# MGI-tech-bioinformatics/SuperPlus

Hardware: AMD Instinct MI355X
Metric: k-mers/s (DF createDict stage: trim + canonical k-mer count + solid filter + spectrum + adjacency) (higher is better)
Workload: dtype u64

## Files before the change

superplus_amd/csrc/dfk.hip:

```cpp
#include "../../include/dfk.h"
#include "dfk_kernels.h"
#include "dfk_arena.h"

#include <algorithm>
#include <chrono>
#include <cstdarg>
#include <cstdio>
#include <cstdlib>
#include <cstring>
#include <atomic>
#include <fcntl.h>
#include <functional>
#include <new>
#include <string>
#include <sys/mman.h>
#include <sys/stat.h>
#include <unistd.h>
#include <condition_variable>
#include <memory>
#include <mutex>
#include <numeric>
#include <thread>
#include <vector>

// ... 201 lines not shown
    }
    DevBuf sums; int rc = c->alloc(sums, nblk * 8, "scan block sums"); if (rc) return rc;
    hipLaunchKernelGGL(k_scan_blocks, dim3((unsigned)nblk), dim3(SCAN_THREADS), 0, c->stream, in, out, n, (uint64_t*)sums.p);
    HIP_TRY(hipGetLastError());
    rc = device_scan(c, (const uint64_t*)sums.p, (uint64_t*)sums.p, nblk); if (rc) return rc;
    hipLaunchKernelGGL(k_scan_add, dim3((unsigned)nblk), dim3(SCAN_THREADS), 0, c->stream, out, n, (const uint64_t*)sums.p);
    HIP_TRY(hipGetLastError());
    HIP_TRY(hipStreamSynchronize(c->stream));
    c->release(sums);
    return 0;
}

struct BucketTable {
    uint32_t log2_nb = 0;
    DevBuf acc;
    DevBuf summ;
    DevBuf classes;
    DevBuf ovf_list; uint64_t n_ovf = 0;
    DevBuf class_hist;
    std::vector<uint64_t> h_class;
    uint64_t n_records = 0, n_inst = 0;
};
struct Partition {
    DevBuf records, base, ipre, items;
    uint64_t n_records = 0, n_inst = 0, n_items = 0;
    uint64_t nb = 0;
};

template <int K>
PartParams part_params(const dfk_ctx* c, uint32_t log2_nb, uint32_t log2_world, int64_t read_id0, uint32_t sub_lo, uint32_t sub_n)
{
    const uint32_t M = c->cfg.minimizer_len;
    return PartParams{M, (uint32_t)K - M + 1, log2_nb, log2_world, read_id0, sub_lo, sub_n,
                      sweep_class_mask(sub_lo, sub_n, log2_nb - log2_world)};
}

int table_totals(dfk_ctx* c, const DevBuf& acc, uint64_t nb, uint64_t* n_records, uint64_t* n_inst)
{
    DevBuf tot; int rc = c->alloc(tot, 16, "bucket totals"); if (rc) return rc;
    HIP_TRY(hipMemsetAsync(tot.p, 0, 16, c->stream));
    hipLaunchKernelGGL(k_sum_acc, dim3(1024), dim3(256), 0, c->stream, (const unsigned long long*)acc.p, nb, (unsigned long long*)tot.p);
    HIP_TRY(hipGetLastError());
    uint64_t h[2];
    HIP_TRY(hipMemcpyAsync(h, tot.p, 16, hipMemcpyDeviceToHost, c->stream));
    HIP_TRY(hipStreamSynchronize(c->stream));
    c->release(tot);
    *n_records = h[0]; *n_inst = h[1];
    return 0;
}

struct ScanJob {
    PartParams pp; ScanPlan plan;
    DevBuf ovf_tmp, d_n;
    DevBuf keys, keys2, fill, sub;
    uint64_t n_pieces = 0; bool count_due = false;
    hipEvent_t ev_scan = nullptr, ev_count = nullptr, ev_part[2] = {nullptr, nullptr};
    std::vector<std::pair<hipEvent_t, hipEvent_t>> ev;
    ~ScanJob()
    {
        for (auto& e : ev) { (void)hipEventDestroy(e.first); (void)hipEventDestroy(e.second); }
        for (hipEvent_t e : {ev_scan, ev_count, ev_part[0], ev_part[1]}) if (e) (void)hipEventDestroy(e);
    }
};

template <int K> bool scan_takes_ranges(const dfk_ctx* c) { return c->cfg.minimizer_len == 16; }

ScanSwitches scan_switches()
// ... 209 lines not shown
    hipLaunchKernelGGL(k_item_flags, dim3(g1), dim3(256), 0, c->stream, (const uint64_t*)P->ipre.p, nb, budget, (uint64_t*)flags.p);
    HIP_TRY(hipGetLastError());
    rc = device_scan(c, (const uint64_t*)flags.p, (uint64_t*)idx.p, nb + 1); if (rc) return rc;
    uint64_t tot[3];
    HIP_TRY(hipMemcpyAsync(&tot[0], (const uint64_t*)P->base.p + nb, 8, hipMemcpyDeviceToHost, c->stream));
    HIP_TRY(hipMemcpyAsync(&tot[1], (const uint64_t*)P->ipre.p + nb, 8, hipMemcpyDeviceToHost, c->stream));
    HIP_TRY(hipMemcpyAsync(&tot[2], (const uint64_t*)idx.p + nb, 8, hipMemcpyDeviceToHost, c->stream));
    HIP_TRY(hipStreamSynchronize(c->stream));
    P->n_records = tot[0]; P->n_inst = tot[1]; P->n_items = tot[2];
    rc = c->alloc(P->items, std::max<uint64_t>(1, P->n_items) * sizeof(ItemRange), "work items"); if (rc) return rc;
    hipLaunchKernelGGL(k_item_pairs, dim3((unsigned)((nb + 255) / 256)), dim3(256), 0, c->stream, (const uint64_t*)flags.p,
                       (const uint64_t*)idx.p, nb, (ItemRange*)P->items.p);
    HIP_TRY(hipGetLastError());
    HIP_TRY(hipStreamSynchronize(c->stream));
    c->release(rec); c->release(inst); c->release(flags); c->release(idx);
    return 0;
}

void release_pass(dfk_ctx* c, Partition* P)
{ c->release(P->records); c->release(P->base); c->release(P->ipre); c->release(P->items); }

template <int K> uint64_t item_budget(const dfk_ctx* c)
{
    constexpr uint64_t S = 1ull << CountCfg<K>::LOG2S;
    if (c->cfg.inst_per_item) return c->cfg.inst_per_item;
    if (c->distinct_per_inst <= 0.0) return 3 * S / 2;
    const double b = 0.367 * (double)S / c->distinct_per_inst;
    return (uint64_t)std::min(std::max(b, 0.5 * (double)S), 3.0 * (double)S);
}

struct ScatterJob { Partition P; DevBuf cur, d_bad; hipStream_t st = nullptr; hipEvent_t e0 = nullptr, e1 = nullptr; uint32_t lo = 0, n = 0; };

template <int K>
int scatter_launch(dfk_ctx* c, const Inputs& in, const BucketTable& T, uint32_t log2_world, int64_t read_id0, ScatterJob* J)
{
    const PartParams pp = part_params<K>(c, T.log2_nb, log2_world, read_id0, J->lo, J->n);
    HIP_TRY(hipEventRecord(J->e0, J->st));
    if (in.n_reads)
        hipLaunchKernelGGL(HIP_KERNEL_NAME(k_scatter_runs<K>), dim3((unsigned)((in.n_reads + 256ull * sweep_reads<K>() - 1) / (256ull * sweep_reads<K>()))),
                           dim3(256), 0, J->st,
                           in.packed, in.packed_bytes, in.base_off, (const uint32_t*)c->good_len.p, in.bc,
                           (int64_t)c->cfg.ign_bc_below, in.n_reads, pp, (const uint4*)T.summ.p, (const uint32_t*)T.classes.p,
                           (unsigned long long*)J->cur.p, J->P.n_records, (uint4*)J->P.records.p);
    HIP_TRY(hipGetLastError());
    HIP_TRY(hipEventRecord(J->e1, J->st));
    return 0;
}

template <int K>
int scatter_begin(dfk_ctx* c, const Inputs& in, const BucketTable& T, uint32_t log2_world, int64_t read_id0,
                  uint32_t sub_lo, uint32_t sub_n, ScatterJob* J, bool launch_now = true)
{
    Partition* P = &J->P;
    J->st = c->stream; J->lo = sub_lo; J->n = sub_n;
    const PartParams pp = part_params<K>(c, T.log2_nb, log2_world, read_id0, sub_lo, sub_n);
    const uint64_t budget = item_budget<K>(c);
    int rc = pass_tables(c, T.acc, T.log2_nb - log2_world, 1u << log2_world, sub_lo, sub_n, budget, P); if (rc) return rc;
    const uint64_t nb = P->nb;
    rc = c->alloc(J->cur, nb * 8, "bucket cursors"); if (rc) return rc;
    rc = c->alloc(P->records, P->n_records * 32, "super-k-mer records"); if (rc) return rc;
    rc = c->alloc(J->d_bad, 16, "scatter check"); if (rc) return rc;
    HIP_TRY(hipMemcpyAsync(J->cur.p, P->base.p, nb * 8, hipMemcpyDeviceToDevice, c->stream));
    HIP_TRY(hipMemsetAsync(J->d_bad.p, 0, 16, c->stream));
    if (!J->e0) { HIP_TRY(hipEventCreate(&J->e0)); HIP_TRY(hipEventCreate(&J->e1)); }
    (void)pp;
    if (launch_now) return scatter_launch<K>(c, in, T, log2_world, read_id0, J);
    return 0;
}

template <int K>
int scatter_end(dfk_ctx* c, const Inputs& in, const BucketTable& T, uint32_t log2_world, int64_t read_id0, ScatterJob* J)
{
    HIP_TRY(hipEventSynchronize(J->e1));
// ... 567 lines not shown
        DevBuf d_n; rc = c->alloc(d_n, 16, "probe counter"); if (rc) return rc;
        HIP_TRY(hipMemsetAsync(d_n.p, 0, 16, c->stream));
        for (const dfk_ctx::Part& pt : c->parts) {
            if (!pt.n) continue;
            if (listed) {
                if (pt.n_blist)
                    hipLaunchKernelGGL(HIP_KERNEL_NAME(k_adjacency_list<K>), dim3((unsigned)std::min<uint64_t>((pt.n_blist + 255) / 256, 16384)), dim3(256), 0,
                                       c->stream, (uint4*)pt.buf.p, (const uint32_t*)((const char*)pt.buf.p + pt.blist + 16), pt.n_blist,
                                       (const SetSlot*)c->set.p, c->set_mask, (unsigned long long*)d_n.p);
            } else
                hipLaunchKernelGGL(HIP_KERNEL_NAME(k_adjacency<K>), dim3((unsigned)std::min<uint64_t>((pt.n + 255) / 256, 8192)), dim3(256), 0,
                                   c->stream, (uint4*)pt.buf.p, pt.n, (const SetSlot*)c->set.p, c->set_mask, (unsigned long long*)d_n.p);
        }
        HIP_TRY(hipGetLastError());
        uint64_t np = 0;
        HIP_TRY(hipMemcpyAsync(&np, d_n.p, 8, hipMemcpyDeviceToHost, c->stream));
        HIP_TRY(hipStreamSynchronize(c->stream));
        c->st.adj_probes = np;
        c->release(d_n); c->release(c->set);
    }
    c->st.ms_adjacency = t.stop();
    TRACE("adjacency done");
    return 0;
}

uint32_t pick_log2_nb(uint64_t n_inst, uint32_t log2_world)
{
    static const uint64_t per = getenv("DFK_INST_PER_BUCKET") ? (uint64_t)atoll(getenv("DFK_INST_PER_BUCKET")) : 850;
    return dfk::pick_log2_nb(n_inst, log2_world, per);
}

PlanInputs plan_inputs(const dfk_ctx* c, const BucketTable& T, const CountRun& R, uint32_t sub_nb, uint32_t lo, bool overlap)
{
    static const double first_div = getenv("DFK_PLAN_FIRST") ? atof(getenv("DFK_PLAN_FIRST")) : 10.0;
    static const double growth = getenv("DFK_PLAN_GROWTH") ? atof(getenv("DFK_PLAN_GROWTH")) : 1.1;
    return PlanInputs{c->budget > c->held ? (double)(c->budget - c->held) : 0.0, sub_nb, lo, T.n_inst, T.n_records, R.inst_seen, R.solid_seen,
                      c->cfg.min_freq, c->seg_attempt, c->plan_derate, overlap, first_div, growth, g_trace};
}

struct StreamSwap {
    dfk_ctx* c; hipStream_t keep;
    StreamSwap(dfk_ctx* ctx, hipStream_t s) : c(ctx), keep(ctx->stream) { c->stream = s; }
    ~StreamSwap() { c->stream = keep; }
};

struct Prescan { BucketTable T; uint64_t n_inst = 0; float ms_trim = 0; };

template <int K>
int run_typed(dfk_ctx* c, const Inputs& in, Prescan* pre = nullptr)
{
    Timer total(c->stream);
    total.start();
    Timer t(c->stream);
    uint64_t n_inst = 0;
    int rc = 0;
    BucketTable T;
    if (pre) { n_inst = pre->n_inst; c->st.ms_trim = pre->ms_trim; T = std::move(pre->T); }
    else {
        t.start();
        TRACE("trim: %llu reads", (unsigned long long)in.n_reads);
        rc = stage_trim<K>(c, in, &n_inst); if (rc) return rc;
        c->st.ms_trim = t.stop();
        TRACE("trim done: %llu instances", (unsigned long long)n_inst);
    }
    c->st.n_reads = in.n_reads; c->st.n_inst = n_inst; c->n_reads = in.n_reads;
    if (!pre) {
        T.log2_nb = pick_log2_nb(n_inst, 0);
        rc = partition_count<K>(c, in, n_inst, 0, 0, &T); if (rc) return rc;
    }
    CountRun R;
    rc = count_run_begin(c, &R); if (rc) return rc;
    c->want_blist = true; c->pending_blist = -1;
    const uint32_t sub_nb = 1u << T.log2_nb;
    const uint32_t forced = (uint32_t)c->cfg.reserved[0];
    const uint32_t per_forced = forced ? std::max<uint32_t>(1, (sub_nb + forced - 1) / forced) : 0;
    const bool overlap = getenv("DFK_NO_OVERLAP") == nullptr;
    uint32_t n_passes = 0, retries = 0;
    c->seg_attempt = 0; c->distinct_per_inst = 0.0;
    struct Job { ScatterJob sj; Arena::PassBlock blk; uint64_t mark = 0; bool valid = false; };
    Job cur, nxt;
    auto drop_events = [&](Job& j) { if (j.sj.e0) { (void)hipEventDestroy(j.sj.e0); (void)hipEventDestroy(j.sj.e1); j.sj.e0 = j.sj.e1 = nullptr; } };
    static const double defer_below = getenv("DFK_DEFER_SWEEP_BELOW") ? atof(getenv("DFK_DEFER_SWEEP_BELOW")) : 1.0;
    auto start = [&](Job& j, uint32_t lo, uint32_t n, bool may_defer = false) -> int {
        j.sj = ScatterJob{}; j.mark = c->alloc_seq; j.valid = false;
        const bool defer = may_defer && (double)n < defer_below * (double)sub_nb;
        TRACE("pass range [%u, %u) of %u (%.1f %%), %.2f GB held of %.2f", lo, lo + n, sub_nb, 100.0 * n / sub_nb, c->held / 1e9, c->budget / 1e9);
        j.blk = Arena::PassBlock{};
        int r = c->alloc(j.blk.block, pass_block_bytes(n, sub_nb, T.n_records), "pass block");
        if (!r) { Arena::Current in_blk(c->arena, j.blk); StreamSwap sw(c, c->stream2); r = scatter_begin<K>(c, in, T, 0, 0, lo, n, &j.sj, !defer); }
        if (r) { (void)hipStreamSynchronize(c->stream2); c->release_since(j.mark); drop_events(j); return r; }
        if (defer) { ScatterJob* sj = &j.sj; c->after_count_launch = [c, &in, &T, sj]() { return scatter_launch<K>(c, in, T, 0, 0, sj); }; TRACE("  (its sweep starts behind k_count)"); }
        j.valid = true;
        return 0;
    };
    auto start_alone = [&](Job& j, uint32_t lo) -> int {
        for (;;) {
            const uint32_t n = forced ? std::min(per_forced, sub_nb - lo) : plan_range(plan_inputs(c, T, R, sub_nb, lo, overlap), c->arena.free_blocks(), nullptr);
            if (!forced && n < sub_nb - lo && (uint64_t)n * 1024 < sub_nb)
                return fail(DFK_E_NOMEM, "HBM budget too small: %.2f GB free of %.2f GB allows passes of %u of %u buckets",
                            (c->budget - c->held) / 1e9, c->budget / 1e9, n, sub_nb);
            const int r = start(j, lo, n);
            if (r != DFK_E_NOMEM || forced || n <= 16 || ++retries > 12) return r;
            c->plan_derate *= 0.7;
            TRACE("out of HBM (%s): planning smaller passes", g_err.c_str());
        }
    };
    rc = start_alone(cur, 0); if (rc) return rc;
    while (cur.valid) {
        const uint32_t lo = cur.sj.lo, n = cur.sj.n, nlo = lo + n;
        rc = scatter_end<K>(c, in, T, 0, 0, &cur.sj); if (rc) return rc;
        const dfk_stats st0 = c->st;
        rc = count_snapshot(c, &R, false); if (rc) return rc;
        { Arena::Current in_blk(c->arena, cur.blk); rc = count_prepare<K>(c, cur.sj.P, R, barcode_words(c, in.bc != nullptr)); }
        nxt.valid = false;
        if (!rc && overlap && nlo < sub_nb) {
            const Partition& P = cur.sj.P;
            (void)P;
            const RunningPass rp{cur.blk.block.bytes, cur.sj.P.n_inst, n, c->arena.offset_of(cur.blk.block)};
            const uint32_t n2 = forced ? std::min(per_forced, sub_nb - nlo) : plan_range(plan_inputs(c, T, R, sub_nb, nlo, overlap), c->arena.free_blocks(), &rp);
            if (n2) {
                const int r2 = start(nxt, nlo, n2, true);
                if (r2 && r2 != DFK_E_NOMEM) return r2;
            }
        }
// ... 698 lines not shown
```

superplus_amd/csrc/dfk_kernels.h:

```cpp
#pragma once
#include <type_traits>
#include "dfk_device.h"
#include "dfk_fallback.h"
#include "dfk_scan_plan.h"

namespace dfk {

template <int K>
__global__ void __launch_bounds__(256)
k_trim(const uint8_t* __restrict__ pq, const uint64_t* __restrict__ pq_off, uint64_t pq_nbytes,
       const uint64_t* __restrict__ base_off, uint64_t packed_bytes, const uint32_t* __restrict__ read_len,
       uint64_t n_reads, uint32_t min_qual, uint32_t* __restrict__ good_len,
       unsigned long long* __restrict__ n_inst, unsigned int* __restrict__ bad,
       unsigned long long* __restrict__ sum_good)
{
    unsigned long long mine = 0, good = 0;
    bool any_bad = false;
    for (uint64_t r = (uint64_t)blockIdx.x * blockDim.x + threadIdx.x; r < n_reads; r += (uint64_t)gridDim.x * blockDim.x) {
        uint32_t gl = 0;
        uint64_t p = pq_off[r], end = pq_off[r + 1];
        uint32_t idx = 0, run = 0;
        const uint64_t b0 = base_off[r], b1 = base_off[r + 1];
        bool ok = p <= end && end <= pq_nbytes && b0 <= b1 && b1 <= packed_bytes && b1 - b0 >= ((uint64_t)read_len[r] + 3) / 4;
        if (!ok) end = p;
// ... 36 lines not shown
        if (gl > rl) gl = rl;
        good_len[r] = gl;
        good += gl;
        if (gl >= (uint32_t)K + 1) mine += gl - K + 1;
    }
    __shared__ unsigned long long sh[2][4];
    __shared__ unsigned int sh_bad;
    if (threadIdx.x == 0) sh_bad = 0;
    __syncthreads();
#pragma unroll
    for (int d = 32; d > 0; d >>= 1) { mine += __shfl_down(mine, d, 64); good += __shfl_down(good, d, 64); }
    if ((threadIdx.x & 63) == 0) { sh[0][threadIdx.x >> 6] = mine; sh[1][threadIdx.x >> 6] = good; }
    if (any_bad) atomicOr(&sh_bad, 1u);
    __syncthreads();
    if (threadIdx.x == 0) {
        unsigned long long a0 = sh[0][0] + sh[0][1] + sh[0][2] + sh[0][3], a1 = sh[1][0] + sh[1][1] + sh[1][2] + sh[1][3];
        if (a0) atomicAdd(n_inst, a0);
        if (a1) atomicAdd(sum_good, a1);
        if (sh_bad) atomicOr(bad, 1u);
    }
}

struct PartParams {
    uint32_t M;
    uint32_t W;
    uint32_t log2_nb;
    uint32_t log2_world;
    int64_t  read_id0;
    uint32_t sub_lo;
    uint32_t sub_n;
    uint32_t class_mask;
};

constexpr uint32_t SWEEP_CLASSES = 32;
__host__ __device__ inline uint32_t sweep_class_of(uint32_t local_bucket, uint32_t log2_local)
{ return log2_local > 5 ? local_bucket >> (log2_local - 5) : local_bucket; }
__host__ __device__ inline uint32_t sweep_class_mask(uint32_t sub_lo, uint32_t sub_n, uint32_t log2_local)
{
    if (sub_n == 0) return 0u;
    const uint32_t a = sweep_class_of(sub_lo, log2_local), b = sweep_class_of(sub_lo + sub_n - 1, log2_local);
    const uint32_t upto_b = b >= 31 ? 0xFFFFFFFFu : ((1u << (b + 1)) - 1u);
    return upto_b & ~((1u << a) - 1u);
}

constexpr uint32_t SUMMARY_OVERFLOW = 15;

__device__ __forceinline__ uint32_t pass_local(uint32_t bucket, const PartParams& pp)
{
    const uint32_t ls = pp.log2_nb - pp.log2_world;
    const uint32_t d = (bucket & ((1u << ls) - 1u)) - pp.sub_lo;
    return d < pp.sub_n ? (bucket >> ls) * pp.sub_n + d : 0xFFFFFFFFu;
}

__device__ __forceinline__ uint32_t bucket_of(uint32_t minhash, const PartParams& pp)
{
    const uint32_t b = (minhash * 0x9E3779B1u) >> (32 - pp.log2_nb);
    return ((b & ((1u << pp.log2_world) - 1u)) << (pp.log2_nb - pp.log2_world)) | (b >> pp.log2_world);
}
constexpr int PART_QCAP = 8;

template <int K>
__device__ __forceinline__ void emit_record(const uint32_t* __restrict__ words, uint64_t n_words, uint64_t bit0,
                                            uint32_t s0, uint32_t nk, uint32_t bucket, uint32_t gl, int32_t tag,
                                            uint64_t dst_index, uint4* __restrict__ records)
{
    const bool hp = s0 > 0;
    const bool hs = s0 + nk + (uint32_t)K <= gl;
    uint64_t bo = bit0 + 2ull * (hp ? s0 - 1 : 0);
    uint64_t wi = bo >> 5; uint32_t sh = (uint32_t)bo & 31u;
    uint32_t w[7];
#pragma unroll
    for (int i = 0; i < 7; ++i) w[i] = (wi + i < n_words) ? words[wi + i] : 0u;
    uint32_t o[6];
#pragma unroll
    for (int i = 0; i < 6; ++i) o[i] = alignbit(w[i + 1], w[i], sh);
    if (!hp) {
#pragma unroll
        for (int i = 5; i > 0; --i) o[i] = (o[i] << 2) | (o[i - 1] >> 30);
// ... 58 lines not shown
    const uint64_t bit0 = byte0 * 8;
    int32_t tag = -1;
    if (bc && (int64_t)r + pp.read_id0 >= ign_bc_below) tag = bc[r];

    const uint32_t mmask = M == 16 ? 0xFFFFFFFFu : ((1u << (2 * M)) - 1u);
    const uint32_t rsh = 2 * (M - 1);
    uint32_t f = 0, rc = 0;
    uint32_t P = 0;
    uint32_t bi = 0;
    uint32_t cur_b = 0, cur_s0 = 0, cur_nk = 0;
    uint32_t qn = 0;

    uint64_t wi = bit0 >> 5;
    uint64_t filled_to = wi;
    auto fill = [&]() {
        uint32_t w[PART_RING];
#pragma unroll
        for (int k = 0; k < PART_RING; ++k) w[k] = filled_to + k < n_words ? words[filled_to + k] : 0u;
#pragma unroll
        for (int k = 0; k < PART_RING; ++k) ring[((filled_to + k) & (PART_RING - 1)) * PART_THREADS + tid] = w[k];
        filled_to += PART_RING;
    };
    uint32_t wbits, wnext = 0;
    if (!WRITE) { fill(); wbits = ring[(wi & (PART_RING - 1)) * PART_THREADS + tid]; }
    else { wbits = wi < n_words ? words[wi] : 0u; wnext = wi + 1 < n_words ? words[wi + 1] : 0u; }
    uint32_t wpos = (uint32_t)bit0 & 31u;
    uint32_t sfx_next = 0xFFFFFFFFu;

    auto close_run = [&]() {
        if (WRITE && cur_b == 0xFFFFFFFFu) return;
        if (!WRITE) {
            if (lh) { const uint32_t bin = class_bin(cur_b, pp); atomicAdd(&lh[bin], 1u); atomicAdd(&lh[(PART_CLASSES << pp.log2_world) + bin], cur_nk); }
            else atomicAdd(&bucket_acc[cur_b], (1ull << 32) | cur_nk);
            cmask |= 1u << sweep_class_of(cur_b & ((1u << log2_local) - 1u), log2_local);
            if (qn < (uint32_t)SUMMARY_RUNS) {
                const uint64_t fld = cur_nk | (cur_rel << 6);
                const uint32_t b = 8u + 12u * qn;
                if (b < 64u) { sum_lo |= fld << b; if (b > 52u) sum_hi |= fld >> (64u - b); }
                else sum_hi |= fld << (b - 64u);
            }
            ++qn;
        } else {
            if (qn == PART_QCAP) {
                for (uint32_t e = 0; e < qn; ++e) {
                    uint32_t a = queue[(2 * e) * PART_THREADS + tid], b = queue[(2 * e + 1) * PART_THREADS + tid];
                    const uint64_t dst = place(b);
                    if (dst != ~0ull) emit_record<K>(words, n_words, bit0, a & 0xFFFFu, a >> 16, b, gl, tag, dst, records);
                }
                qn = 0;
            }
            queue[(2 * qn) * PART_THREADS + tid] = cur_s0 | (cur_nk << 16);
            queue[(2 * qn + 1) * PART_THREADS + tid] = cur_b;
            ++qn;
        }
    };

    for (uint32_t j = 0; j < gl; ++j) {
        uint32_t b = (wbits >> wpos) & 3u;
        wpos += 2;
        if (wpos == 32) {
            wpos = 0; ++wi;
            if (!WRITE) { if (wi == filled_to) fill(); wbits = ring[(wi & (PART_RING - 1)) * PART_THREADS + tid]; }
            else { wbits = wnext; wnext = wi + 1 < n_words ? words[wi + 1] : 0u; }
        }
        f = ((f << 2) | b) & mmask;
        rc = (rc >> 2) | ((3u - b) << rsh);
        if (j + 1 < M) continue;
        uint32_t h = mmer_hash(f < rc ? f : rc);
// ... 12 lines not shown
            if (open) {
                if (s != 0) close_run();
                cur_b = bucket; cur_s0 = s; cur_nk = 1;
                if (!WRITE) cur_rel = older ? (uint32_t)sidx[(bi + 1) * PART_THREADS + tid] - bi - 1u : W - 1u - bi + Pi;
            } else ++cur_nk;
        }
        arr[bi * PART_THREADS + tid] = h;
        if (++bi == W) {
            uint32_t run = h, ri = W - 1;
            if (!WRITE) sidx[(W - 1) * PART_THREADS + tid] = (uint8_t)(W - 1);
            for (int i0 = (int)W - 2; i0 >= 0; i0 -= 8) {
                uint32_t v[8];
#pragma unroll
                for (int k = 0; k < 8; ++k) v[k] = i0 - k >= 0 ? arr[(i0 - k) * PART_THREADS + tid] : 0u;
#pragma unroll
                for (int k = 0; k < 8; ++k) {
                    const int i = i0 - k;
                    if (i >= 0) {
                        const bool lt = v[k] < run;
                        run = lt ? v[k] : run;
                        arr[i * PART_THREADS + tid] = run;
                        if (!WRITE) { ri = lt ? (uint32_t)i : ri; sidx[i * PART_THREADS + tid] = (uint8_t)ri; }
                    }
                }
            }
            bi = 0;
        }
        if (bi + 1 < W) sfx_next = arr[(bi + 1) * PART_THREADS + tid];
    }
    close_run();
    if (!WRITE) {
        const uint64_t lo = sum_lo | (qn <= (uint32_t)SUMMARY_RUNS ? qn : SUMMARY_OVERFLOW), hi = sum_hi;
        summaries[r] = uint4{(uint32_t)lo, (uint32_t)(lo >> 32), (uint32_t)hi, (uint32_t)(hi >> 32)};
        if (read_classes) read_classes[r] = cmask;
        if (qn > (uint32_t)SUMMARY_RUNS && bucket_cur) {
            const unsigned long long at = atomicAdd(bucket_cur, 1ull);
            if (at < n_out) reinterpret_cast<uint32_t*>(records)[at] = (uint32_t)r;
        }
    }
    if (WRITE) {
        for (uint32_t e = 0; e < qn; ++e) {
            uint32_t a = queue[(2 * e) * PART_THREADS + tid], b = queue[(2 * e + 1) * PART_THREADS + tid];
            const uint64_t dst = place(b);
            if (dst != ~0ull) emit_record<K>(words, n_words, bit0, a & 0xFFFFu, a >> 16, b, gl, tag, dst, records);
        }
    }
}

template <int K, bool WRITE>
__global__ void __launch_bounds__(PART_THREADS)
k_partition(const uint8_t* __restrict__ packed, uint64_t packed_bytes, const uint64_t* __restrict__ base_off,
            const uint32_t* __restrict__ good_len, const int32_t* __restrict__ bc, int64_t ign_bc_below,
            uint64_t n_reads, PartParams pp,
            unsigned long long* __restrict__ bucket_acc,
            unsigned long long* __restrict__ class_hist,
            unsigned long long* __restrict__ bucket_cur,
            uint64_t n_out,
            uint4* __restrict__ records,
            uint4* __restrict__ summaries,
            const uint32_t* __restrict__ read_list,
            uint64_t n_list,
            const uint64_t* __restrict__ slice_base,
            uint32_t* __restrict__ read_classes)
{
    extern __shared__ uint32_t smem[];
    uint32_t* lh = nullptr;
    const uint32_t n_bins = 2u * (PART_CLASSES << pp.log2_world);
// ... 88 lines not shown
#pragma unroll
                for (int k = 0; k < NW; ++k) {
                    const uint64_t i = wi + k;
                    const uint32_t v = words[i < n_words ? i : n_words - 1];
                    w[k] = i < n_words ? v : 0u;
                }
            };
            uint64_t nbit = bit0 + 2 * (M - 1);
            uint32_t nw[NW];
            load(nbit, nw);
            uint32_t f = 0, rc = 0;
            {
                const uint64_t wi = bit0 >> 5;
                const uint32_t w0 = words[wi < n_words ? wi : n_words - 1], w1 = words[wi + 1 < n_words ? wi + 1 : n_words - 1];
                const uint32_t pw = alignbit(wi + 1 < n_words ? w1 : 0u, wi < n_words ? w0 : 0u, (uint32_t)bit0 & 31u);
#pragma unroll
                for (int j = 0; j < M - 1; ++j) { const uint32_t b = (pw >> (2 * j)) & 3u; f = ((f << 2) | b) & mmask; rc = (rc >> 2) | ((3u - b) << rsh); }
            }
            const uint32_t n_mmers = gl - M + 1;
            uint32_t arr[W], sidxw[(W + 3) / 4];
            auto sidx_get = [&](int i) -> uint32_t { return (sidxw[i >> 2] >> (8 * (i & 3))) & 255u; };
            auto sidx_set = [&](int i, uint32_t v) { const uint32_t sh = 8u * (uint32_t)(i & 3); sidxw[i >> 2] = (sidxw[i >> 2] & ~(255u << sh)) | (v << sh); };
#pragma unroll
            for (int i = 0; i < (W + 3) / 4; ++i) sidxw[i] = 0;
            uint32_t P = 0, Pi = 0;
            uint32_t cur_b = 0, cur_nk = 0, cur_rel = 0;
            auto close_run = [&]() {
                if (qn < (uint32_t)RUNS) {
                    runb[qn * PART_THREADS + tid] = cur_b;
                    runf[qn * PART_THREADS + tid] = (uint16_t)(cur_nk | (cur_rel << 6));
                } else {
                    if (lh) { const uint32_t bin = class_bin(cur_b, pp); atomicAdd(&lh[bin], 1u); atomicAdd(&lh[(PART_CLASSES << pp.log2_world) + bin], cur_nk); }
                    else atomicAdd(&bucket_acc[cur_b], (1ull << 32) | cur_nk);
                    cmask |= 1u << sweep_class_of(cur_b & ((1u << log2_local) - 1u), log2_local);
                }
                ++qn;
            };
            for (uint32_t t0 = 0; t0 < n_mmers; t0 += W) {
                uint32_t a[NA];
                {
                    const uint32_t sh = (uint32_t)nbit & 31u;
#pragma unroll
                    for (int i = 0; i < NA; ++i) a[i] = alignbit(i + 1 < NW ? nw[i + 1] : 0u, nw[i], sh);
                }
                nbit += 2 * W;
                load(nbit, nw);
                static_for<0, W>([&](auto bi_c) {
                    constexpr int bi = decltype(bi_c)::value;
                    if (t0 + (uint32_t)bi < n_mmers) {
                        const uint32_t b = (a[(2 * bi) >> 5] >> ((2 * bi) & 31)) & 3u;
                        f = ((f << 2) | b) & mmask;
                        rc = (rc >> 2) | ((3u - b) << rsh);
                        const uint32_t h = mmer_hash(f < rc ? f : rc);
                        const bool newmin = bi == 0 || h < P;
                        P = newmin ? h : P;
                        Pi = newmin ? (uint32_t)bi : Pi;
                        const bool first = t0 == 0;
                        if (!first || bi == W - 1) {
                            uint32_t mv = P;
                            bool older = false;
                            if constexpr (bi != W - 1) { older = arr[bi + 1] < mv; mv = older ? arr[bi + 1] : mv; }
                            const uint32_t bucket = bucket_of(mv, pp);
                            const bool open = first || bucket != cur_b || cur_nk == (uint32_t)KTraits<K>::NK_MAX;
                            if (open && !first) close_run();
                            const uint32_t rel = (bi != W - 1 && older) ? sidx_get(bi + 1 < W ? bi + 1 : 0) - (uint32_t)bi - 1u : (uint32_t)(W - 1 - bi) + Pi;
                            cur_rel = open ? rel : cur_rel;
                            cur_nk = open ? 1u : cur_nk + 1u;
                            cur_b = open ? bucket : cur_b;
                        }
                        arr[bi] = h;
                        if (bi == W - 1) {
                            uint32_t run = h, ri = W - 1;
                            sidx_set(W - 1, W - 1);
                            static_for<0, W - 1>([&](auto j_c) {
                                constexpr int i = W - 2 - decltype(j_c)::value;
                                const bool lt = arr[i] < run; run = lt ? arr[i] : run; arr[i] = run; ri = lt ? (uint32_t)i : ri; sidx_set(i, ri);
                            });
                        }
                    }
                });
            }
            close_run();
        }
        const uint32_t mine = min(qn, (uint32_t)RUNS);
        for (uint32_t i = 0; KEYS ? __syncthreads_or(i < mine) != 0 : __ballot(i < mine) != 0ull; ++i) {
            const bool has = i < mine;
            uint32_t cb = 0, nk = 0;
            if (has) {
                cb = runb[i * PART_THREADS + tid];
                const uint64_t fld = runf[i * PART_THREADS + tid];
                nk = (uint32_t)fld & 63u;
                const uint32_t bfld = 8u + 12u * i;
                if (bfld < 64u) { sum_lo |= fld << bfld; if (bfld > 52u) sum_hi |= fld >> (64u - bfld); } else sum_hi |= fld << (bfld - 64u);
                if constexpr (!KEYS) {
                    if (lh) { const uint32_t bin = class_bin(cb, pp); atomicAdd(&lh[bin], 1u); atomicAdd(&lh[(PART_CLASSES << pp.log2_world) + bin], nk); }
                    else atomicAdd(&bucket_acc[cb], (1ull << 32) | nk);
                }
                cmask |= 1u << sweep_class_of(cb & ((1u << log2_local) - 1u), log2_local);
            }
            if constexpr (KEYS) {
                const uint64_t m = __ballot(has);
                if (m) {
                    const uint32_t rk = __builtin_amdgcn_mbcnt_hi((uint32_t)(m >> 32), __builtin_amdgcn_mbcnt_lo((uint32_t)m, 0u));
                    const int lead = __ffsll((unsigned long long)m) - 1;
                    uint32_t at = 0;
                    if (has && rk == 0) at = atomicAdd(st_n, (uint32_t)__popcll(m));
                    at = __shfl(at, lead) + rk;
                    if (has) {
                        const uint32_t cls = cb >> sk.ib;
                        st_key[at] = ((cb & ((1u << sk.ib) - 1u)) << 6) | nk;
                        st_cls[at] = (uint8_t)cls;
                        atomicAdd(&st_h[cls], 1u);
                    }
                }
                __syncthreads();
                if (*st_n > (uint32_t)(SCAN_STAGE - PART_THREADS)) flush();
            }
        }
        if (r < n_reads) {
            const uint64_t lo = sum_lo | (qn <= (uint32_t)SUMMARY_RUNS ? qn : SUMMARY_OVERFLOW);
            summaries[r] = uint4{(uint32_t)lo, (uint32_t)(lo >> 32), (uint32_t)sum_hi, (uint32_t)(sum_hi >> 32)};
            if (read_classes) read_classes[r] = cmask;
        }
        if (qn > (uint32_t)SUMMARY_RUNS) {
            const unsigned long long at = atomicAdd(ovf_count, 1ull);
            if (at < ovf_cap) ovf_list[at] = (uint32_t)r;
        }
    }
    if constexpr (KEYS) { __syncthreads(); if (*st_n) flush(); }
    if (lh) {
        __syncthreads();
        for (uint32_t i = threadIdx.x; i < n_bins; i += PART_THREADS) if (lh[i]) atomicAdd(&class_hist[i], (unsigned long long)lh[i]);
    }
}

constexpr int KEY_VECS = 4;
static_assert(KEY_TILE == 256u * 4u * KEY_VECS, "a tile is KEY_VECS 16-byte vectors per thread of a 256-thread block");
__device__ __forceinline__ uint32_t key_vec_n(uint64_t t0, uint64_t t1, int j)
{
    const uint64_t i = t0 + ((uint64_t)j * 256u + threadIdx.x) * 4u;
    return i < t1 ? (uint32_t)min((uint64_t)4, t1 - i) : 0u;
}
__device__ __forceinline__ void key_tile_load(const uint32_t* __restrict__ k, uint64_t t0, uint64_t t1, uint4 (&v)[KEY_VECS])
{
#pragma unroll
    for (int j = 0; j < KEY_VECS; ++j) {
        const uint64_t i = t0 + ((uint64_t)j * 256u + threadIdx.x) * 4u;
        v[j] = i < t1 ? *reinterpret_cast<const uint4*>(k + i) : make_uint4(0u, 0u, 0u, 0u);
    }
}
template <typename F>
__device__ __forceinline__ void key_tile_each(uint64_t t0, uint64_t t1, const uint4 (&v)[KEY_VECS], F&& f)
{
#pragma unroll
    for (int j = 0; j < KEY_VECS; ++j) {
// ... 123 lines not shown
            y = ((y >> 1) & 0x55555555u) | ((y & 0x55555555u) << 1);
            const uint32_t fw = y >> (32 - 2 * M), rcv = ~x & mmask;
            const uint32_t bucket = bucket_of(mmer_hash(fw < rcv ? fw : rcv), pp);
            const uint32_t lb = pass_local(bucket, pp);
            if (lb != 0xFFFFFFFFu) f(s0, nk, lb, bucket >> (pp.log2_nb - pp.log2_world), bit0, (uint32_t)i + 1 == n);
            s0 += nk;
        }
    }
}

template <int K>
__global__ void __launch_bounds__(256)
k_scatter_slices(const uint8_t* __restrict__ packed, uint64_t packed_bytes, const uint64_t* __restrict__ base_off,
                 const uint32_t* __restrict__ good_len, const int32_t* __restrict__ bc, int64_t ign_bc_below,
                 uint64_t n_reads, PartParams pp, const uint4* __restrict__ summaries, const uint32_t* __restrict__ read_classes,
                 const uint64_t* __restrict__ slice_base,
                 unsigned long long* __restrict__ slice_fill,
                 uint4* __restrict__ records)
{
    __shared__ uint32_t cnt[256];
    __shared__ unsigned long long at[256];
    __shared__ uint16_t list[256 * SLICE_READS];
    __shared__ uint32_t n_list;
    const uint32_t world = 1u << pp.log2_world;
    const int lane = threadIdx.x & 63;
    const uint64_t r_block = (uint64_t)blockIdx.x * 256 * SLICE_READS;
    if (threadIdx.x < world) cnt[threadIdx.x] = 0;
    if (threadIdx.x == 0) n_list = 0;
    __syncthreads();
#pragma unroll
    for (int j = 0; j < SLICE_READS; ++j) {
        const uint32_t rel = 256u * j + threadIdx.x;
        const uint64_t r = r_block + rel;
        const bool hit = r < n_reads && (!read_classes || (read_classes[r] & pp.class_mask) != 0u);
        const unsigned long long mk = __ballot(hit);
        uint32_t w = 0;
        if (lane == 0 && mk) w = atomicAdd(&n_list, (uint32_t)__popcll(mk));
        w = __builtin_amdgcn_readfirstlane(w);
        if (hit) list[w + __popcll(mk & ((1ull << lane) - 1ull))] = (uint16_t)rel;
    }
    __syncthreads();
    const uint32_t n = n_list;
    for (uint32_t i = threadIdx.x; i < n; i += 256)
        for_each_run_in_pass<K, false>(r_block + list[i], packed, packed_bytes, base_off, pp, summaries,
                                       [&](uint32_t, uint32_t, uint32_t, uint32_t owner, uint64_t, bool) { atomicAdd(&cnt[owner], 1u); });
    __syncthreads();
    if (threadIdx.x < world) {
        const uint32_t m = cnt[threadIdx.x];
        at[threadIdx.x] = slice_base[threadIdx.x] + (m ? atomicAdd(&slice_fill[threadIdx.x], (unsigned long long)m) : 0ull);
        cnt[threadIdx.x] = 0;
    }
    __syncthreads();
    const uint32_t* words = reinterpret_cast<const uint32_t*>(packed);
    const uint64_t n_words = (packed_bytes + 3) >> 2;
    (void)good_len;
    for (uint32_t i = threadIdx.x; i < n; i += 256) {
        const uint64_t r = r_block + list[i];
        int32_t tag = -1;
        if (bc && (int64_t)r + pp.read_id0 >= ign_bc_below) tag = bc[r];
        for_each_run_in_pass<K, true>(r, packed, packed_bytes, base_off, pp, summaries,
            [&](uint32_t s0, uint32_t nk, uint32_t lb, uint32_t owner, uint64_t bit0, bool last) {
                const uint64_t dst = at[owner] + atomicAdd(&cnt[owner], 1u);
                if (dst < slice_base[owner + 1]) emit_record<K>(words, n_words, bit0, s0, nk, lb, last ? 0u : 0xFFFFFFFFu, tag, dst, records);
            });
    }
}

#ifndef DFK_SWEEP_READS
#define DFK_SWEEP_READS 8
#endif
template <int K> constexpr int sweep_reads() { return KTraits<K>::KW == 4 ? 2 : DFK_SWEEP_READS; }
template <int K>
__global__ void __launch_bounds__(256)
k_scatter_runs(const uint8_t* __restrict__ packed, uint64_t packed_bytes, const uint64_t* __restrict__ base_off,
               const uint32_t* __restrict__ good_len, const int32_t* __restrict__ bc, int64_t ign_bc_below,
               uint64_t n_reads, PartParams pp, const uint4* __restrict__ summaries, const uint32_t* __restrict__ read_classes,
               unsigned long long* __restrict__ bucket_cur, uint64_t n_out, uint4* __restrict__ records)
{
    constexpr int SWEEP_READS = sweep_reads<K>();
    __shared__ uint16_t list[256 * SWEEP_READS];
    __shared__ uint32_t n_list;
    (void)good_len;
    const int lane = threadIdx.x & 63;
    const uint64_t r_block = (uint64_t)blockIdx.x * 256 * SWEEP_READS;
    if (threadIdx.x == 0) n_list = 0;
    __syncthreads();
#pragma unroll
    for (int j = 0; j < SWEEP_READS; ++j) {
        const uint32_t rel = 256u * j + threadIdx.x;
        const uint64_t r = r_block + rel;
        const bool hit = r < n_reads && (read_classes[r] & pp.class_mask) != 0u;
        const unsigned long long mk = __ballot(hit);
        uint32_t at = 0;
        if (lane == 0 && mk) at = atomicAdd(&n_list, (uint32_t)__popcll(mk));
        at = __builtin_amdgcn_readfirstlane(at);
        if (hit) list[at + __popcll(mk & ((1ull << lane) - 1ull))] = (uint16_t)rel;
    }
    __syncthreads();
    const uint32_t n = n_list;
    const uint32_t* words = reinterpret_cast<const uint32_t*>(packed);
    const uint64_t n_words = (packed_bytes + 3) >> 2;
    for (uint32_t i = threadIdx.x; i < n; i += 256) {
        const uint64_t r = r_block + list[i];
        int32_t tag = -1;
        if (bc && (int64_t)r + pp.read_id0 >= ign_bc_below) tag = bc[r];
        for_each_run_in_pass<K, true>(r, packed, packed_bytes, base_off, pp, summaries,
            [&](uint32_t s0, uint32_t nk, uint32_t lb, uint32_t, uint64_t bit0, bool last) {
                const uint64_t dst = atomicAdd(&bucket_cur[lb], 1ull);
                if (dst < n_out) emit_record<K>(words, n_words, bit0, s0, nk, lb, last ? 0u : 0xFFFFFFFFu, tag, dst, records);
            });
    }
}



struct CountParams {
    uint32_t min_freq, min_bc;
    uint32_t n_items;
    uint32_t single;
    uint64_t seg_cap;
    uint32_t do_adj;
    uint32_t keep_pre;
};

struct CountGlobals {
    unsigned long long n_distinct;
    unsigned long long big_cursor;
    unsigned int next_item;
    unsigned int n_overflow;
    unsigned int solid_overflow;
    unsigned int n_split;
    unsigned long long n_boundary;
    unsigned long long part_cursor;
    unsigned int n_wg_idle;
    unsigned int pad_idle;
};

constexpr int COUNT_HIST_BINS = 256;
constexpr uint32_t COUNT_MAX_PROBE = 96;
constexpr uint32_t HIST_GLOBAL_BINS = 1u << 24;
constexpr uint32_t FLAG_SOLID = 0x80000000u;

template <int K> struct WaveStage {
// ... 1445 lines not shown
```

superplus_amd/csrc/dfk_scan_plan.h:

```cpp
#pragma once
#include <algorithm>
#include <cstddef>
#include <cstdint>
#include <vector>
#include "dfk_fallback.h"

namespace dfk {

constexpr int PART_THREADS = 128;
constexpr int PART_RING = 2;
constexpr int SUMMARY_RUNS = 10;
constexpr uint32_t PART_CLASSES = 64;

struct ScanKeys {
    uint32_t* keys;
    unsigned long long* fill;
    uint64_t cap;
    uint32_t ib;
};
constexpr int SCAN_STAGE = 1536;
constexpr uint32_t KEY_SUB_BITS = 14;
constexpr size_t SCAN_RUN_LDS = (sizeof(uint32_t) + sizeof(uint16_t)) * SUMMARY_RUNS * PART_THREADS;
constexpr size_t SCAN_STAGE_LDS = (sizeof(uint32_t) + 1) * SCAN_STAGE + (sizeof(unsigned long long) + sizeof(uint32_t)) * PART_CLASSES + sizeof(uint32_t);
static_assert(SCAN_RUN_LDS + SCAN_STAGE_LDS <= 16384, "ten scan blocks a CU (160 KB of LDS)");

constexpr uint64_t SCAN_TAIL_READS = 32ull << 20;
constexpr uint64_t KEY_SCRATCH_MAX = 16ull << 30;
constexpr uint32_t SCAN_BLOCKS_PER_CU = 128;

struct ScanSwitches {
    bool key_piece_set = false; uint64_t key_piece = 0;
    uint64_t key_tail = SCAN_TAIL_READS;
    uint32_t scan_blocks = 0;
    bool no_overlap = false;
};

struct ScanInputs {
    int K; uint32_t W, log2_nb, log2_world;
    uint64_t n_reads, packed_bytes;
    bool by_class;
    bool register_scan;
    bool second_stream;
    ScanSwitches sw;
};
// ... 109 lines not shown
```

Baseline: 64.67 billion.

## Encode per-run bucket codes in read class words so sweep emits only matching runs

Replaces the per-read 32-class bitmask with a word that stores a 4-bit coarse bucket code for each of the first seven runs, plus quarter flags for the remaining runs. The scatter sweep now builds a per-run candidate list and decodes a single run directly from the summary, instead of re-walking every run of every hit read. This is meant to cut redundant run decoding and hashing in multi-pass scatter. It also adds dynamic LDS to the deferred sweep launched beside k_count, presumably to limit co-residency, and retunes the plan's first-pass divisor and growth. The costs are extra candidate-list overflow loops and block syncs, and overflow reads now get a zero class word.

```diff
diff --git a/superplus_amd/csrc/dfk.hip b/superplus_amd/csrc/dfk.hip
--- a/superplus_amd/csrc/dfk.hip
+++ b/superplus_amd/csrc/dfk.hip
@@ -257,7 +257,7 @@
 {
     const uint32_t M = c->cfg.minimizer_len;
     return PartParams{M, (uint32_t)K - M + 1, log2_nb, log2_world, read_id0, sub_lo, sub_n,
-                      sweep_class_mask(sub_lo, sub_n, log2_nb - log2_world)};
+                      sweep_pass_set(sub_lo, sub_n, log2_nb - log2_world)};
 }
 
 int table_totals(dfk_ctx* c, const DevBuf& acc, uint64_t nb, uint64_t* n_records, uint64_t* n_inst)
@@ -533,13 +533,13 @@
 struct ScatterJob { Partition P; DevBuf cur, d_bad; hipStream_t st = nullptr; hipEvent_t e0 = nullptr, e1 = nullptr; uint32_t lo = 0, n = 0; };
 
 template <int K>
-int scatter_launch(dfk_ctx* c, const Inputs& in, const BucketTable& T, uint32_t log2_world, int64_t read_id0, ScatterJob* J)
+int scatter_launch(dfk_ctx* c, const Inputs& in, const BucketTable& T, uint32_t log2_world, int64_t read_id0, ScatterJob* J, bool beside_count = false)
 {
     const PartParams pp = part_params<K>(c, T.log2_nb, log2_world, read_id0, J->lo, J->n);
     HIP_TRY(hipEventRecord(J->e0, J->st));
     if (in.n_reads)
         hipLaunchKernelGGL(HIP_KERNEL_NAME(k_scatter_runs<K>), dim3((unsigned)((in.n_reads + 256ull * sweep_reads<K>() - 1) / (256ull * sweep_reads<K>()))),
-                           dim3(256), 0, J->st,
+                           dim3(256), beside_count ? sweep_lds_beside_count<K>() : 0, J->st,
                            in.packed, in.packed_bytes, in.base_off, (const uint32_t*)c->good_len.p, in.bc,
                            (int64_t)c->cfg.ign_bc_below, in.n_reads, pp, (const uint4*)T.summ.p, (const uint32_t*)T.classes.p,
                            (unsigned long long*)J->cur.p, J->P.n_records, (uint4*)J->P.records.p);
@@ -1173,8 +1173,8 @@
 
 PlanInputs plan_inputs(const dfk_ctx* c, const BucketTable& T, const CountRun& R, uint32_t sub_nb, uint32_t lo, bool overlap)
 {
-    static const double first_div = getenv("DFK_PLAN_FIRST") ? atof(getenv("DFK_PLAN_FIRST")) : 10.0;
-    static const double growth = getenv("DFK_PLAN_GROWTH") ? atof(getenv("DFK_PLAN_GROWTH")) : 1.1;
+    static const double first_div = getenv("DFK_PLAN_FIRST") ? atof(getenv("DFK_PLAN_FIRST")) : 20.0;
+    static const double growth = getenv("DFK_PLAN_GROWTH") ? atof(getenv("DFK_PLAN_GROWTH")) : 1.5;
     return PlanInputs{c->budget > c->held ? (double)(c->budget - c->held) : 0.0, sub_nb, lo, T.n_inst, T.n_records, R.inst_seen, R.solid_seen,
                       c->cfg.min_freq, c->seg_attempt, c->plan_derate, overlap, first_div, growth, g_trace};
 }
@@ -1230,7 +1230,7 @@
         int r = c->alloc(j.blk.block, pass_block_bytes(n, sub_nb, T.n_records), "pass block");
         if (!r) { Arena::Current in_blk(c->arena, j.blk); StreamSwap sw(c, c->stream2); r = scatter_begin<K>(c, in, T, 0, 0, lo, n, &j.sj, !defer); }
         if (r) { (void)hipStreamSynchronize(c->stream2); c->release_since(j.mark); drop_events(j); return r; }
-        if (defer) { ScatterJob* sj = &j.sj; c->after_count_launch = [c, &in, &T, sj]() { return scatter_launch<K>(c, in, T, 0, 0, sj); }; TRACE("  (its sweep starts behind k_count)"); }
+        if (defer) { ScatterJob* sj = &j.sj; c->after_count_launch = [c, &in, &T, sj]() { return scatter_launch<K>(c, in, T, 0, 0, sj, true); }; TRACE("  (its sweep starts behind k_count)"); }
         j.valid = true;
         return 0;
     };
diff --git a/superplus_amd/csrc/dfk_kernels.h b/superplus_amd/csrc/dfk_kernels.h
--- a/superplus_amd/csrc/dfk_kernels.h
+++ b/superplus_amd/csrc/dfk_kernels.h
@@ -92,18 +92,6 @@
     uint32_t class_mask;
 };
 
-constexpr uint32_t SWEEP_CLASSES = 32;
-__host__ __device__ inline uint32_t sweep_class_of(uint32_t local_bucket, uint32_t log2_local)
-{ return log2_local > 5 ? local_bucket >> (log2_local - 5) : local_bucket; }
-__host__ __device__ inline uint32_t sweep_class_mask(uint32_t sub_lo, uint32_t sub_n, uint32_t log2_local)
-{
-    if (sub_n == 0) return 0u;
-    const uint32_t a = sweep_class_of(sub_lo, log2_local), b = sweep_class_of(sub_lo + sub_n - 1, log2_local);
-    const uint32_t upto_b = b >= 31 ? 0xFFFFFFFFu : ((1u << (b + 1)) - 1u);
-    return upto_b & ~((1u << a) - 1u);
-}
-
-constexpr uint32_t SUMMARY_OVERFLOW = 15;
 
 __device__ __forceinline__ uint32_t pass_local(uint32_t bucket, const PartParams& pp)
 {
@@ -228,8 +216,8 @@
         if (!WRITE) {
             if (lh) { const uint32_t bin = class_bin(cur_b, pp); atomicAdd(&lh[bin], 1u); atomicAdd(&lh[(PART_CLASSES << pp.log2_world) + bin], cur_nk); }
             else atomicAdd(&bucket_acc[cur_b], (1ull << 32) | cur_nk);
-            cmask |= 1u << sweep_class_of(cur_b & ((1u << log2_local) - 1u), log2_local);
             if (qn < (uint32_t)SUMMARY_RUNS) {
+                cmask = sweep_word_add(cmask, qn, cur_b & ((1u << log2_local) - 1u), log2_local);
                 const uint64_t fld = cur_nk | (cur_rel << 6);
                 const uint32_t b = 8u + 12u * qn;
                 if (b < 64u) { sum_lo |= fld << b; if (b > 52u) sum_hi |= fld >> (64u - b); }
@@ -308,7 +296,7 @@
     if (!WRITE) {
         const uint64_t lo = sum_lo | (qn <= (uint32_t)SUMMARY_RUNS ? qn : SUMMARY_OVERFLOW), hi = sum_hi;
         summaries[r] = uint4{(uint32_t)lo, (uint32_t)(lo >> 32), (uint32_t)hi, (uint32_t)(hi >> 32)};
-        if (read_classes) read_classes[r] = cmask;
+        if (read_classes) read_classes[r] = qn <= (uint32_t)SUMMARY_RUNS ? cmask : 0u;
         if (qn > (uint32_t)SUMMARY_RUNS && bucket_cur) {
             const unsigned long long at = atomicAdd(bucket_cur, 1ull);
             if (at < n_out) reinterpret_cast<uint32_t*>(records)[at] = (uint32_t)r;
@@ -463,7 +451,7 @@
                 } else {
                     if (lh) { const uint32_t bin = class_bin(cur_b, pp); atomicAdd(&lh[bin], 1u); atomicAdd(&lh[(PART_CLASSES << pp.log2_world) + bin], cur_nk); }
                     else atomicAdd(&bucket_acc[cur_b], (1ull << 32) | cur_nk);
-                    cmask |= 1u << sweep_class_of(cur_b & ((1u << log2_local) - 1u), log2_local);
+                    { const uint32_t lbk = cur_b & ((1u << log2_local) - 1u); cmask |= 1u << (log2_local > 5 ? lbk >> (log2_local - 5) : lbk); }
                 }
                 ++qn;
             };
@@ -527,7 +515,7 @@
                     if (lh) { const uint32_t bin = class_bin(cb, pp); atomicAdd(&lh[bin], 1u); atomicAdd(&lh[(PART_CLASSES << pp.log2_world) + bin], nk); }
                     else atomicAdd(&bucket_acc[cb], (1ull << 32) | nk);
                 }
-                cmask |= 1u << sweep_class_of(cb & ((1u << log2_local) - 1u), log2_local);
+                cmask = sweep_word_add(cmask, i, cb & ((1u << log2_local) - 1u), log2_local);
             }
             if constexpr (KEYS) {
                 const uint64_t m = __ballot(has);
@@ -551,7 +539,7 @@
         if (r < n_reads) {
             const uint64_t lo = sum_lo | (qn <= (uint32_t)SUMMARY_RUNS ? qn : SUMMARY_OVERFLOW);
             summaries[r] = uint4{(uint32_t)lo, (uint32_t)(lo >> 32), (uint32_t)sum_hi, (uint32_t)(sum_hi >> 32)};
-            if (read_classes) read_classes[r] = cmask;
+            if (read_classes) read_classes[r] = qn <= (uint32_t)SUMMARY_RUNS ? cmask : 0u;
         }
         if (qn > (uint32_t)SUMMARY_RUNS) {
             const unsigned long long at = atomicAdd(ovf_count, 1ull);
@@ -741,7 +729,7 @@
     for (int j = 0; j < SLICE_READS; ++j) {
         const uint32_t rel = 256u * j + threadIdx.x;
         const uint64_t r = r_block + rel;
-        const bool hit = r < n_reads && (!read_classes || (read_classes[r] & pp.class_mask) != 0u);
+        const bool hit = r < n_reads && (!read_classes || sweep_word_candidates(read_classes[r], pp.class_mask) != 0u);
         const unsigned long long mk = __ballot(hit);
         uint32_t w = 0;
         if (lane == 0 && mk) w = atomicAdd(&n_list, (uint32_t)__popcll(mk));
@@ -779,6 +767,7 @@
 #define DFK_SWEEP_READS 8
 #endif
 template <int K> constexpr int sweep_reads() { return KTraits<K>::KW == 4 ? 2 : DFK_SWEEP_READS; }
+template <int K> constexpr unsigned sweep_lds_beside_count() { return KTraits<K>::KW == 4 ? 0u : 2048u; }
 template <int K>
 __global__ void __launch_bounds__(256)
 k_scatter_runs(const uint8_t* __restrict__ packed, uint64_t packed_bytes, const uint64_t* __restrict__ base_off,
@@ -787,37 +776,86 @@
                unsigned long long* __restrict__ bucket_cur, uint64_t n_out, uint4* __restrict__ records)
 {
     constexpr int SWEEP_READS = sweep_reads<K>();
-    __shared__ uint16_t list[256 * SWEEP_READS];
+    constexpr uint32_t CAP = 256u * SWEEP_READS;
+    static_assert(CAP <= 4096 && SUMMARY_RUNS <= 16, "an entry is 12 bits of read and 4 of run");
+    __shared__ uint16_t list[CAP];
     __shared__ uint32_t n_list;
     (void)good_len;
     const int lane = threadIdx.x & 63;
-    const uint64_t r_block = (uint64_t)blockIdx.x * 256 * SWEEP_READS;
-    if (threadIdx.x == 0) n_list = 0;
-    __syncthreads();
-#pragma unroll
-    for (int j = 0; j < SWEEP_READS; ++j) {
-        const uint32_t rel = 256u * j + threadIdx.x;
-        const uint64_t r = r_block + rel;
-        const bool hit = r < n_reads && (read_classes[r] & pp.class_mask) != 0u;
-        const unsigned long long mk = __ballot(hit);
-        uint32_t at = 0;
-        if (lane == 0 && mk) at = atomicAdd(&n_list, (uint32_t)__popcll(mk));
-        at = __builtin_amdgcn_readfirstlane(at);
-        if (hit) list[at + __popcll(mk & ((1ull << lane) - 1ull))] = (uint16_t)rel;
-    }
-    __syncthreads();
-    const uint32_t n = n_list;
+    const uint64_t r_block = (uint64_t)blockIdx.x * CAP;
     const uint32_t* words = reinterpret_cast<const uint32_t*>(packed);
     const uint64_t n_words = (packed_bytes + 3) >> 2;
-    for (uint32_t i = threadIdx.x; i < n; i += 256) {
-        const uint64_t r = r_block + list[i];
-        int32_t tag = -1;
-        if (bc && (int64_t)r + pp.read_id0 >= ign_bc_below) tag = bc[r];
-        for_each_run_in_pass<K, true>(r, packed, packed_bytes, base_off, pp, summaries,
-            [&](uint32_t s0, uint32_t nk, uint32_t lb, uint32_t, uint64_t bit0, bool last) {
-                const uint64_t dst = atomicAdd(&bucket_cur[lb], 1ull);
-                if (dst < n_out) emit_record<K>(words, n_words, bit0, s0, nk, lb, last ? 0u : 0xFFFFFFFFu, tag, dst, records);
-            });
+    const uint32_t M = pp.M;
+    const uint32_t mmask = M == 16 ? 0xFFFFFFFFu : ((1u << (2 * M)) - 1u);
+    uint32_t cw[SWEEP_READS];
+#pragma unroll
+    for (int j = 0; j < SWEEP_READS; ++j) {
+        const uint64_t r = r_block + 256u * j + threadIdx.x;
+        cw[j] = r < n_reads ? read_classes[r] : 0u;
+    }
+    if (threadIdx.x == 0) n_list = 0;
+    __syncthreads();
+    uint32_t j = 0;
+    uint32_t m = sweep_word_candidates(cw[0], pp.class_mask);
+    for (;;) {
+        bool full = false;
+        for (;;) {
+            const uint32_t c = (uint32_t)__popc(m);
+            const uint32_t incl = wave_incl_scan(c, lane);
+            const uint32_t tot = (uint32_t)__builtin_amdgcn_readlane((int)incl, 63);
+            uint32_t at = 0;
+            if (lane == 0 && tot) at = atomicAdd(&n_list, tot);
+            at = uniform32(at);
+            uint32_t pos = at + incl - c;
+            while (__ballot(m != 0u && pos < CAP) != 0ull)
+                if (m != 0u && pos < CAP) { list[pos++] = (uint16_t)(((256u * j + threadIdx.x) << 4) | (uint32_t)(__ffs((int)m) - 1)); m &= m - 1u; }
+            __syncthreads();
+            full = n_list > CAP;
+            if (full || ++j == (uint32_t)SWEEP_READS) break;
+            uint32_t w = 0;
+#pragma unroll
+            for (int k = 1; k < SWEEP_READS; ++k) w = j == (uint32_t)k ? cw[k] : w;
+            m = sweep_word_candidates(w, pp.class_mask);
+        }
+        const uint32_t n = min(n_list, CAP);
+        for (uint32_t i = threadIdx.x; i < n; i += 256) {
+            const uint32_t e = list[i], ri = e & 15u;
+            const uint64_t r = r_block + (e >> 4);
+            const uint4 sm = summaries[r];
+            const uint64_t bit0 = base_off[r] * 8;
+            const uint32_t cnt = sm.x & 15u;
+            if (sweep_candidate_exists(ri, cnt)) {
+                const uint64_t lo = (uint64_t)sm.x | ((uint64_t)sm.y << 32), hi = (uint64_t)sm.z | ((uint64_t)sm.w << 32);
+                uint32_t s0 = 0, fld = 0;
+#pragma unroll
+                for (int q = 0; q < SUMMARY_RUNS; ++q) {
+                    constexpr int B0 = 8;
+                    const int b = B0 + 12 * q;
+                    const uint32_t f = (uint32_t)(b + 12 <= 64 ? lo >> b : b >= 64 ? hi >> (b - 64) : (lo >> b) | (hi << (64 - b))) & 0xFFFu;
+                    s0 += (uint32_t)q < ri ? f & 63u : 0u;
+                    fld = (uint32_t)q == ri ? f : fld;
+                }
+                const uint32_t nk = fld & 63u, rel = fld >> 6;
+                const uint64_t bo = bit0 + 2ull * (s0 + rel);
+                const uint64_t wi = bo >> 5;
+                const uint32_t w0 = words[wi], w1 = wi + 1 < n_words ? words[wi + 1] : 0u;
+                const uint32_t x = alignbit(w1, w0, (uint32_t)bo & 31u) & mmask;
+                uint32_t y = __brev(x);
+                y = ((y >> 1) & 0x55555555u) | ((y & 0x55555555u) << 1);
+                const uint32_t fw = y >> (32 - 2 * M), rcv = ~x & mmask;
+                const uint32_t lb = pass_local(bucket_of(mmer_hash(fw < rcv ? fw : rcv), pp), pp);
+                if (lb != 0xFFFFFFFFu) {
+                    int32_t tag = -1;
+                    if (bc && (int64_t)r + pp.read_id0 >= ign_bc_below) tag = bc[r];
+                    const uint64_t dst = atomicAdd(&bucket_cur[lb], 1ull);
+                    if (dst < n_out) emit_record<K>(words, n_words, bit0, s0, nk, lb, ri + 1u == cnt ? 0u : 0xFFFFFFFFu, tag, dst, records);
+                }
+            }
+        }
+        if (!full) break;
+        __syncthreads();
+        if (threadIdx.x == 0) n_list = 0;
+        __syncthreads();
     }
 }
 
diff --git a/superplus_amd/csrc/dfk_scan_plan.h b/superplus_amd/csrc/dfk_scan_plan.h
--- a/superplus_amd/csrc/dfk_scan_plan.h
+++ b/superplus_amd/csrc/dfk_scan_plan.h
@@ -10,6 +10,34 @@
 constexpr int PART_THREADS = 128;
 constexpr int PART_RING = 2;
 constexpr int SUMMARY_RUNS = 10;
+constexpr uint32_t SUMMARY_OVERFLOW = 15;
+
+constexpr uint32_t SWEEP_CODED_RUNS = 7;
+constexpr uint32_t SWEEP_CODES = 15;
+constexpr uint32_t sweep_code_of(uint32_t local_bucket, uint32_t log2_local) { return 1u + ((local_bucket * SWEEP_CODES) >> log2_local); }
+constexpr uint32_t sweep_quarter_of(uint32_t local_bucket, uint32_t log2_local) { return (local_bucket << 2) >> log2_local; }
+constexpr uint32_t sweep_pass_set(uint32_t sub_lo, uint32_t sub_n, uint32_t log2_local)
+{
+    if (sub_n == 0) return 0u;
+    const uint32_t last = sub_lo + sub_n - 1;
+    const uint32_t codes = (2u << sweep_code_of(last, log2_local)) - (1u << sweep_code_of(sub_lo, log2_local));
+    const uint32_t quarters = (2u << sweep_quarter_of(last, log2_local)) - (1u << sweep_quarter_of(sub_lo, log2_local));
+    return codes | (quarters << 16);
+}
+constexpr uint32_t sweep_word_add(uint32_t word, uint32_t run, uint32_t local_bucket, uint32_t log2_local)
+{
+    return run < SWEEP_CODED_RUNS ? word | (sweep_code_of(local_bucket, log2_local) << (4u * run))
+                                  : word | (1u << (28u + sweep_quarter_of(local_bucket, log2_local)));
+}
+constexpr uint32_t sweep_word_candidates(uint32_t word, uint32_t set)
+{
+    uint32_t m = 0;
+    for (uint32_t i = 0; i < SWEEP_CODED_RUNS; ++i) m |= ((set >> ((word >> (4u * i)) & 15u)) & 1u) << i;
+    if ((word >> 28) & (set >> 16)) m |= ((1u << (SUMMARY_RUNS - SWEEP_CODED_RUNS)) - 1u) << SWEEP_CODED_RUNS;
+    return m;
+}
+constexpr bool sweep_candidate_exists(uint32_t run, uint32_t count) { return count != SUMMARY_OVERFLOW && run < count; }
+
 constexpr uint32_t PART_CLASSES = 64;
 
 struct ScanKeys {
```

New measurement: 65.30 billion, median of 6. No clear change (+1.0%).
